# kfirc1503/generative-audio

Hardware: AMD Instinct MI355X
Metric: spectrogram-frames/sec, NPPC K=5 FullSubNet+ train step (higher is better)
Workload: dtype bf16

## Files before the change

generative-audio_amd/csrc/tcn.hip:

```cpp
#include <cstdlib>
#include "common.h"
#include "mfma_tile.h"
#include "nppc_hip.h"

namespace {


template <typename T, int EPI>
__global__ __launch_bounds__(256) void gemm_nt_kernel(GemmArgs g) {
  const int ks = g.ksplit > 1 ? g.ksplit : 1;
  const int z = blockIdx.z / ks, ksl = blockIdx.z % ks;
  const T* A = reinterpret_cast<const T*>(g.A) + (size_t)z * g.strideA + (size_t)ksl * g.K;
  const T* B = reinterpret_cast<const T*>(g.B) + (size_t)z * g.strideB + (size_t)ksl * g.K;
  const int lane = threadIdx.x & 63, wave = threadIdx.x >> 6, n = lane & 15, q = lane >> 4;
  const int r0 = blockIdx.x * 128 + wave * 32, c0 = blockIdx.y * 64;
  const T* ap = A + (size_t)(r0 + n) * g.lda + 8 * q;
  const T* bp = B + (size_t)(c0 + n) * g.ldb + 8 * q;
  f32x4 acc[2][4];
  nt_reg_mainloop<T>(acc, g.K / 32, g.lda, g.ldb, [&](int kk) { return ap + 32 * kk; }, [&](int kk) { return bp + 32 * kk; },
                     g.relu_in);

  const NtEpilogue<T, EPI> ep(g, z, blockIdx.x * 128);
  float s1 = 0.f, s2 = 0.f;
#pragma unroll
// ... 488 lines not shown

extern "C" int nppc_gemm_nt_splitk(int prec, const void* A, long lda, const void* B, long ldb, float* C, long ldc, int M, int N,
                                   long K, int ksplit, void* stream) {
  if (!A || !B || !C || M <= 0 || N <= 0 || K <= 0 || ksplit < 1) return NPPC_EBADARG;
  const int bk = prec == NPPC_PREC_BF16 ? 64 : 32;
  if (M % 128 || N % 128 || K % ((long)bk * ksplit) || lda % 8 || ldb % 8) return NPPC_EUNSUPPORTED;
  dim3 grid(M / 128, N / 128, ksplit);
  LAUNCH_T(prec, gemm_nt_tiled_kernel, grid, (const TT*)A, lda, (const TT*)B, ldb, C, ldc, (long)M * ldc, K / ksplit);
  return NPPC_OK;
}

namespace {

typedef __attribute__((ext_vector_type(4))) short s16x4;

template <int BN>
__global__ __launch_bounds__(256, 2) void gemm_tn_tiled_kernel(const bf16_t* __restrict__ A, long lda, const bf16_t* __restrict__ B,
                                                               long ldb, float* __restrict__ C, long ldc, long slab_stride,
                                                               long Rz, int ntap, int Wp, int shift_a, int nzb, long bsA,
                                                               long bsB, long bsC) {
  constexpr int BM = 128, BR = 64, NT = 2 * BM;
  constexpr int RSA = BM + 8, RSB = BN + 8;
  constexpr int WN = BN / 2;
  constexpr int NJ = WN / 16;
  __shared__ __attribute__((aligned(16))) bf16_t lds[2][BR * RSA + BR * RSB];
  const int tid = threadIdx.x, lane = tid & 63, wave = tid >> 6, i16 = lane & 15, qq = lane >> 4;
  const int wm = wave >> 1, wn = wave & 1;
  unsigned bx = blockIdx.x, by = blockIdx.y, bz = blockIdx.z;
  if (gridDim.z % 8 == 0) {
    const unsigned tiles = gridDim.x * gridDim.y;
    const unsigned lin = bx + gridDim.x * (by + gridDim.y * bz);
    const unsigned xcd = lin & 7, j = lin >> 3;
    bz = xcd + 8 * (j / tiles);
    const unsigned t = j % tiles;
    bx = t % gridDim.x;
    by = t / gridDim.x;
  }
  const unsigned bb = bz / nzb;
  bz %= nzb;
  A += (size_t)bb * bsA;
  B += (size_t)bb * bsB;
  C += (size_t)bb * bsC;
  const long m0 = (long)bx * BM, n0 = (long)by * BN;
  const int ksl = nzb / ntap, tap = bz / ksl;
  const long rbase = (long)(bz % ksl) * Rz;
  const long boff = ntap == 9 ? (long)(tap / 3 - 1) * Wp + (tap % 3 - 1) : 0;
  const bf16_t* Ab = A + (rbase + (shift_a ? boff : 0)) * lda + m0;
  const bf16_t* Bb = B + (rbase + (shift_a ? 0 : boff)) * ldb + n0;
  float* Cz = C + (size_t)bz * slab_stride;

  constexpr int ACH = BM / 8, BCH = BN / 8;
  constexpr int NA = BR * ACH / NT, NB = BR * BCH / NT;
  static_assert(NA == 4 && (NB == 4 || NB == 2 || NB == 1), "staging slots are named registers");
  const int arow = tid / ACH, ac = tid % ACH, brow = tid / BCH, bc = tid % BCH;
  constexpr int ASTEP = NT / ACH, BSTEP = NT / BCH;
  const bf16_t* gA = Ab + (long)arow * lda + ac * 8;
  const bf16_t* gB = Bb + (long)brow * ldb + bc * 8;
  const int sA = arow * RSA + ac * 8, sB = BR * RSA + brow * RSB + bc * 8;
  uint4 ra0, ra1, ra2, ra3, rb0, rb1 = {}, rb2 = {}, rb3 = {};
#define TN_GLOAD(r0)                                                            \
  ra0 = *reinterpret_cast<const uint4*>(gA + ((r0) + 0 * ASTEP) * lda);         \
  ra1 = *reinterpret_cast<const uint4*>(gA + ((r0) + 1 * ASTEP) * lda);         \
  ra2 = *reinterpret_cast<const uint4*>(gA + ((r0) + 2 * ASTEP) * lda);         \
  ra3 = *reinterpret_cast<const uint4*>(gA + ((r0) + 3 * ASTEP) * lda);         \
  rb0 = *reinterpret_cast<const uint4*>(gB + ((r0) + 0 * BSTEP) * ldb);         \
  if (NB >= 2) rb1 = *reinterpret_cast<const uint4*>(gB + ((r0) + 1 * BSTEP) * ldb); \
  if (NB == 4) {                                                                \
    rb2 = *reinterpret_cast<const uint4*>(gB + ((r0) + 2 * BSTEP) * ldb);       \
    rb3 = *reinterpret_cast<const uint4*>(gB + ((r0) + 3 * BSTEP) * ldb);       \
  }
#define TN_LSTORE(buf)                                                          \
  *reinterpret_cast<uint4*>(&lds[buf][sA + 0 * ASTEP * RSA]) = ra0;             \
  *reinterpret_cast<uint4*>(&lds[buf][sA + 1 * ASTEP * RSA]) = ra1;             \
  *reinterpret_cast<uint4*>(&lds[buf][sA + 2 * ASTEP * RSA]) = ra2;             \
  *reinterpret_cast<uint4*>(&lds[buf][sA + 3 * ASTEP * RSA]) = ra3;             \
  *reinterpret_cast<uint4*>(&lds[buf][sB + 0 * BSTEP * RSB]) = rb0;             \
  if (NB >= 2) *reinterpret_cast<uint4*>(&lds[buf][sB + 1 * BSTEP * RSB]) = rb1; \
  if (NB == 4) {                                                                \
    *reinterpret_cast<uint4*>(&lds[buf][sB + 2 * BSTEP * RSB]) = rb2;           \
    *reinterpret_cast<uint4*>(&lds[buf][sB + 3 * BSTEP * RSB]) = rb3;           \
  }
  auto tfrag = [&](const bf16_t* tile, int rs, int r0, int col0) -> bf16x8 {
    const int q4 = i16 >> 2, p4 = i16 & 3;
    const bf16_t* base = tile + (r0 + 8 * qq + q4) * rs + col0 + 4 * p4;
    const s16x4 lo = __builtin_amdgcn_ds_read_tr16_b64_v4i16((__attribute__((address_space(3))) s16x4*)(base));
    const s16x4 hi = __builtin_amdgcn_ds_read_tr16_b64_v4i16((__attribute__((address_space(3))) s16x4*)(base + 4 * rs));
    typedef __attribute__((ext_vector_type(8))) short s16x8;
    s16x8 v = {lo[0], lo[1], lo[2], lo[3], hi[0], hi[1], hi[2], hi[3]};
    return __builtin_bit_cast(bf16x8, v);
  };

  f32x4 acc[4][NJ];
#pragma unroll
  for (int i = 0; i < 4; ++i)
#pragma unroll
    for (int j = 0; j < NJ; ++j) acc[i][j] = f32x4{0.f, 0.f, 0.f, 0.f};

  const long nstage = Rz / BR;
  TN_GLOAD(0)
  TN_LSTORE(0)
  __syncthreads();
  for (long s = 0; s < nstage; ++s) {
    const int buf = (int)(s & 1);
    if (s + 1 < nstage) { TN_GLOAD((s + 1) * BR) }
    const bf16_t* ta = lds[buf];
    const bf16_t* tb = lds[buf] + BR * RSA;
#pragma unroll
    for (int ks = 0; ks < BR / 32; ++ks) {
      bf16x8 af[4], bfr[NJ];
#pragma unroll
      for (int i = 0; i < 4; ++i) af[i] = tfrag(ta, RSA, 32 * ks, wm * 64 + 16 * i);
#pragma unroll
      for (int j = 0; j < NJ; ++j) bfr[j] = tfrag(tb, RSB, 32 * ks, wn * WN + 16 * j);
#pragma unroll
      for (int i = 0; i < 4; ++i)
#pragma unroll
        for (int j = 0; j < NJ; ++j) acc[i][j] = mma16(af[i], bfr[j], acc[i][j]);
    }
    if (s + 1 < nstage) { TN_LSTORE(buf ^ 1) }
    __syncthreads();
  }
#undef TN_GLOAD
#undef TN_LSTORE
#pragma unroll
  for (int i = 0; i < 4; ++i)
#pragma unroll
    for (int j = 0; j < NJ; ++j)
#pragma unroll
      for (int r = 0; r < 4; ++r) {
        const long row = m0 + wm * 64 + 16 * i + 4 * qq + r;
        const long col = n0 + wn * WN + 16 * j + i16;
        Cz[row * ldc + col] = acc[i][j][r];
      }
}

}

namespace {
constexpr int DR_BM = 256;

__device__ __forceinline__ int dr_key(int row, int nch) {
  const int k = (row & 3) | (((row >> 3) & 1) << 2);
  return nch >= 8 ? k : (k & (nch - 1));
}
__device__ __forceinline__ int dr_phys(int bytes_in_row, int key, int nch) {
  const int c = bytes_in_row >> 5;
  int pc = c + key;
  if (pc >= nch) pc -= nch;
// ... 132 lines not shown
    for (int j = 0; j < NJ; ++j)
#pragma unroll
      for (int r = 0; r < 4; ++r) {
        const long row = m0 + wm * (BM / 4) + 16 * i + 4 * qq + r;
        const long col = c0 + wn * (BN / 2) + 16 * j + i16;
        Cz[row * ldc + col] = acc[i][j][r];
      }
  if (do_rowsum && i16 == 0) {
#pragma unroll
    for (int i = 0; i < MI; ++i)
#pragma unroll
      for (int r = 0; r < 4; ++r) rs[m0 + wm * (BM / 4) + 16 * i + 4 * qq + r] = racc[i][r];
  }
}

__device__ __forceinline__ void dr_xcd_remap(unsigned& bx, unsigned& by, unsigned& bz) {
  if (gridDim.z % 8 == 0) {
    const unsigned tiles = gridDim.x * gridDim.y;
    const unsigned lin = bx + gridDim.x * (by + gridDim.y * bz);
    const unsigned xcd = lin & 7, j = lin >> 3;
    bz = xcd + 8 * (j / tiles);
    const unsigned t = j % tiles;
    bx = t % gridDim.x;
    by = t / gridDim.x;
  }
}

template <int BN, int BR, int STAGES>
__global__ __launch_bounds__(512, 1) void gemm_tn_dma_kernel(const bf16_t* __restrict__ A, long lda, const bf16_t* __restrict__ B,
                                                             long ldb, float* __restrict__ C, long ldc, long slab_stride, long Rz,
                                                             int nzb, long bsA, long bsB, long bsC, float* __restrict__ rowsum,
                                                             int ntap, int Wp, int shift_a) {
  unsigned bx = blockIdx.x, by = blockIdx.y, bz = blockIdx.z;
  dr_xcd_remap(bx, by, bz);
  const unsigned bb = bz / nzb;
  bz %= nzb;
  A += (size_t)bb * bsA;
  B += (size_t)bb * bsB;
  C += (size_t)bb * bsC;
  const int ksl = nzb / ntap, tap = bz / ksl;
  const long boff = ntap == 9 ? (long)(tap / 3 - 1) * Wp + (tap % 3 - 1) : 0;
  const long rbase = (long)(bz % ksl) * Rz;
  float* rs = rowsum != nullptr && by == 0 ? rowsum + ((size_t)bb * nzb + bz) * ((size_t)gridDim.x * DR_BM) : nullptr;
  dma_tile<DR_BM, BN, BR, STAGES>(A, lda, B, ldb, C + (size_t)bz * slab_stride, ldc, (long)bx * DR_BM, (long)by * BN, (long)by * BN,
                           rbase + (shift_a ? boff : 0), rbase + (shift_a ? 0 : boff), Rz, rs);
}

template <int BM, int BR, int STAGES>
__global__ __launch_bounds__(512, 1) void gemm_tn_dma2_kernel(const bf16_t* __restrict__ A, long lda, const bf16_t* __restrict__ B1,
                                                              long ldb1, int nt1, const bf16_t* __restrict__ B2, long ldb2, int N2,
                                                              float* __restrict__ C, long ldc, long slab_stride, long Rz,
                                                              float* __restrict__ rowsum) {
  unsigned bx = blockIdx.x, by = blockIdx.y, bz = blockIdx.z;
  dr_xcd_remap(bx, by, bz);
  const long m0 = (long)bx * BM, rbase = (long)bz * Rz;
  float* Cz = C + (size_t)bz * slab_stride;
  float* rs = rowsum != nullptr && by == 0 ? rowsum + (size_t)bz * ((size_t)gridDim.x * BM) : nullptr;
  if ((int)by >= nt1 && N2 == 64) {
    dma_tile<BM, 64, BR, STAGES>(A, lda, B2, ldb2, Cz, ldc, m0, 0, (long)nt1 * 192, rbase, rbase, Rz, nullptr);
    return;
  }
  const bool second = (int)by >= nt1;
  const long n0 = (long)(second ? by - nt1 : by) * 192;
  dma_tile<BM, 192, BR, STAGES>(A, lda, second ? B2 : B1, second ? ldb2 : ldb1, Cz, ldc, m0, n0, (long)by * 192, rbase, rbase, Rz, rs);
}

}

static int launch_tn(const void* A, long lda, const void* B, long ldb, float* C, long ldc, int M, int N, long R, int ksplit,
// ... 88 lines not shown
      return NPPC_ELAUNCH;
    attr = true;
  }
  hipLaunchKernelGGL((gemm_tn_dma2_kernel<DR_BM, 32, 5>), dim3(M / DR_BM, nt1 + nt2, ksplit), dim3(512), smem, s, (const bf16_t*)A,
                     lda, (const bf16_t*)B1, ldb1, nt1, (const bf16_t*)B2, ldb2, N2, C, ldc, (long)M * ldc, R / ksplit, rowsum);
  NPPC_CHECK_LAUNCH();
  return NPPC_OK;
}

extern "C" int nppc_gemm_tn_splitk_batched(const void* A, long lda, long sA, const void* B, long ldb, long sB, float* C, long ldc,
                                           long sC, int M, int N, long R, int ksplit, int batch, void* stream) {
  if (batch < 1) return NPPC_EBADARG;
  return launch_tn(A, lda, B, ldb, C, ldc, M, N, R, ksplit, 1, 0, 0, stream, batch, sA, sB, sC);
}

extern "C" int nppc_gemm_tn_splitk_taps(const void* A, long lda, const void* B, long ldb, float* C, long ldc, int M, int N,
                                        long R, int ksplit, int Wp, int shift_a, void* stream) {
  return launch_tn(A, lda, B, ldb, C, ldc, M, N, R, ksplit, 9, Wp, shift_a, stream);
}
```

generative-audio_amd/nppc_audio/_hip.py:

```python
import ctypes
import os
import threading

import torch

_HERE = os.path.dirname(os.path.abspath(__file__))
LIB_PATH = os.path.join(_HERE, "libnppc_hip.so")

PREC_BF16 = 0
PREC_F32 = 1
_ERR = {1: "bad argument", 2: "kernel launch failed", 3: "unsupported shape/configuration"}

_lib = None

c_p = ctypes.c_void_p
c_i = ctypes.c_int
c_l = ctypes.c_long
c_f = ctypes.c_float


def lib():
    global _lib
    if _lib is None:
        if not os.path.exists(LIB_PATH):
# ... 17 lines not shown


def stream():
    return c_p(torch.cuda.current_stream().cuda_stream)


def check(rc, what):
    if rc != 0:
        raise RuntimeError(f"{what} failed: {_ERR.get(rc, rc)}")


def ptr_array(tensors):
    for t in tensors:
        assert t.is_cuda and t.is_contiguous()
    return (ctypes.c_void_p * len(tensors))(*[t.data_ptr() for t in tensors])


def mid_bwd_part_elems(B, C, Tp, batch):
    n = c_l()
    call("nppc_tcn_mid_bwd_part_elems", B, C, Tp, batch, ctypes.byref(n))
    return n.value


def conv_thin_part_elems():
    n = c_l()
    call("nppc_conv_thin_part_elems", ctypes.byref(n))
    return n.value


def masked_mse_work_elems():
# ... 57 lines not shown
                           I, I, I, I, I, I, P],
    "nppc_scale_transpose": [I, P, P, P, I, I, I, I, I, I, P],
    "nppc_gemm_nt": [I, I, P, L, L, P, L, L, P, L, L, P, L, P, L, L, P, L, P, L, I, I, I, I, I, I, I, I, I, P],
    "nppc_tcn_mid_bwd_part_elems": [I, I, I, I, PL],
    "nppc_tcn_mid_bwd": [I, P, P, P, P, P, P, P, P, P, P, P, P, P, P, P, P, P, P, P, P, P, P, P, P, P, P, I, I, I, P,
                         I, I, I, I, I, F, L, L, L, I, I, P],
    "nppc_tcn_mid_bwd_finish": [P, L, P, L, I, I, I, P, P, P, P, P, P, P, P, P, P, I, I, L, L, I, I, P],
    "nppc_gemm_nt_colsum": [I, I, P, L, L, P, L, L, P, L, L, P, L, P, L, L, I, I, I, I, I, I, I, P, P],
    "nppc_gemm_nt_gn": [I, P, L, L, P, L, L, P, L, L, P, P, L, P, L, L, P, L, D, F, I, I, I, I, I, I, I, P],
    "nppc_tcn_pack_sconv": [I, P, P, P, P, P, P, P, I, I, I, I, I, I, L, L, L, L, P],
    "nppc_gemm_nt_splitk": [I, P, L, P, L, P, L, I, I, L, I, P],
    "nppc_gemm_tn_splitk": [P, L, P, L, P, L, I, I, L, I, P],
    "nppc_gemm_tn_splitk_rowsum": [P, L, P, L, P, L, I, I, L, I, P, P],
    "nppc_gemm_tn_splitk2": [P, L, P, L, I, P, L, I, P, L, I, L, I, P, P],
    "nppc_gemm_tn_splitk_batched": [P, L, L, P, L, L, P, L, L, I, I, L, I, I, P],
    "nppc_reduce_slabs_t": [P, I, L, L, P, L, I, I, L, L, I, P],
    "nppc_gemm_tn_splitk_taps": [P, L, P, L, P, L, I, I, L, I, I, I, P],
    "nppc_tcn_dwconv": [I, P, P, P, P, P, P, P, P, P, I, I, I, I, I, I, F, L, L, L, I, P],
    "nppc_tcn_gn_apply": [I, P, P, P, P, P, I, I, I, I, I, F, L, L, L, I, P],
    "nppc_pack_matrix": [I, P, P, I, I, I, I, I, P],
    "nppc_pack_matrix_batched": [I, P, P, I, I, I, I, I, I, I, L, L, L, L, P],
    "nppc_subband_mean": [I, P, I, P, I, L, P, P, P, I, I, I, I, I, P],
    "nppc_subband_stage": [I, P, I, P, I, L, P, P, I, I, I, I, I, I, I, I, P],
    "nppc_sb_head": [I, P, P, P, P, L, I, I, I, I, I, P],
    "nppc_gram": [P, P, P, P, P, I, I, L, P],
    "nppc_combine": [P, P, P, P, P, P, P, I, I, L, P],
    "nppc_gs_solve": [P, P, P, I, I, I, P],
    "nppc_gs_bwd_solve": [P, P, P, P, I, I, I, P],
    "nppc_loss_solve": [P, P, P, P, P, P, P, P, P, P, I, I, P],
    "nppc_loss_bwd_coef": [P, P, P, F, F, P, I, I, P],
# ... 176 lines not shown
```

generative-audio_amd/nppc_audio/engine.py:

```python
import ctypes

import numpy as np
import torch

from . import _hip as H
from .ops_lstm import (PackedLSTM, PackedLSTMBwd, ROW_PAD, WGRAD_SPLITS, bwd_head_fusable, forward_x_ld, lstm2_backward, lstm2_forward,
                       own_workspaces, padded_rows,
                       rows_view, workspace)

TCN_HIDDEN = 512
TCN_DILATIONS = (1, 2, 5, 9, 1, 2, 5, 9)
BRANCHES = ("", "_real", "_imag")
EPI_PLAIN, EPI_PRELU_STATS, EPI_RESIDUAL, EPI_RELU, EPI_PLAIN_F32, EPI_MASK_POS = 0, 1, 2, 3, 4, 5


def rup(a, b):
    return (a + b - 1) // b * b


TCN_WGRAD_SPLITS = 8
TCN_WGRAD_MAIN_BLOCKS = 1


class FlatParams:

    def __init__(self, module, device):
        named = list(module.named_parameters())
        total = sum(p.numel() for _, p in named)
        self.flat = torch.empty(total, dtype=torch.float32, device=device)
        self.grad = None
        self.off = {}
        o = 0
        for n, p in named:
            k = p.numel()
            self.flat[o:o + k].copy_(p.detach().reshape(-1))
            p.data = self.flat[o:o + k].view(p.shape)
# ... 63 lines not shown
        self.F, self.nm, self.O = num_freqs, n_maps, out_size
        self.nb, self.la, self.Hd, self.G = sb_neighbors, look_ahead, sb_hidden, groups
        self.ks = tuple(kersize)
        self.prec = prec
        self.dt = H.dtype_of(prec)
        self.trainable = trainable
        self.C = n_maps * num_freqs
        self.ldC = rup(self.C, 64)
        self.ldF = rup(num_freqs, 64)
        self.KC = self.ldC
        self.dev = flat.flat.device
        self.I = 2 * sb_neighbors + 1 + 3
        self.sP = flat.branch_stride()
        self.sAtt = flat.attention_stride()
        self.packed_version = None
        self._side = None
        self._gen = 0
        self.last_train = None
        self.grad_range_hook = None
        self.early_buckets_ok = self._check_bucket_layout() if trainable else False
        self.pre_lstm_hook = None
        self.defer_join = False
        self.join_pending = False
        self.bufs = {}
        own_workspaces(self)
        self.lstm = PackedLSTM(self.I, self.Hd, prec, self.dev)
        self.KX = self.lstm.kx
        self.mult = torch.from_numpy(unfold_multiplicity(self.F, self.nb)).to(self.dev)
        C, ldC, ldF = self.C, self.ldC, self.ldF
        self.W1p = torch.zeros(8, 3, TCN_HIDDEN, ldC, dtype=self.dt, device=self.dev)
# ... 227 lines not shown
            self.last_train = d
        return out

    def _grad_buffer(self):
        first = self.fp.named[0][1]
        for k in (0, 1):
            if self.gbuf[k] is None:
                self.gbuf[k] = torch.empty_like(self.fp.flat)
            if first.grad is None or first.grad.data_ptr() != self.gbuf[k].data_ptr():
                self.fp.grad = self.gbuf[k]
                return self.gbuf[k]
        raise RuntimeError("unreachable")

    def g(self, name):
        return self.fp.gview(name)

    def _wgrad(self, AT, lda, sA, BT, ldb, sB, rows, ncolsN, K, S, dst_name_or_tensor, dst_ld, out_rows, ncols, slab,
               batch=1, sDst=0, permH=0, col0=0, accumulate=0):
        s = H.stream()
        dst = self.g(dst_name_or_tensor) if isinstance(dst_name_or_tensor, str) else dst_name_or_tensor
        bk = 64 if self.prec == H.PREC_BF16 else 32
        if batch == 1 and rows % 128 == 0 and ncolsN % 128 == 0 and K % (bk * S) == 0:
            H.call("nppc_gemm_nt_splitk", self.prec, AT, lda, BT, ldb, slab, ncolsN, rows, ncolsN, K, S, s)
        else:
            H.call("nppc_gemm_nt", self.prec, EPI_PLAIN_F32, AT, lda, sA, BT, ldb, sB, slab, ncolsN, rows * ncolsN, None,
                   0, None, 0, 0, None, 0, None, 0, rows, ncolsN, K, rows, rows, ncolsN, 0, batch, S, s)
        H.call("nppc_reduce_slabs", slab, S, rows * ncolsN, ncolsN, dst, dst_ld, out_rows, col0, ncols, permH, accumulate,
               S * rows * ncolsN, sDst, batch, s)

    def _lstm_wgrad(self, dg1, dg2, x_rows, h1_rows, h2_rows, Tv, Nseq, head=None, guards=None):
# ... 130 lines not shown
        self._side.wait_stream(main)
        with torch.cuda.stream(self._side):
            self._lstm_wgrad(dg1, dg2, d["x_rows"], lo["h1_rows"], lo["h2_rows"], Tv, Nseq, head=head_wgrad,
                             guards=(lo["h1_guard"], lo["h2_guard"]) if "h1_guard" in lo else None)
            if self.grad_range_hook is not None and self.early_buckets_ok:
                self.grad_range_hook(G, self.fp.off["sb_model.sequence_model.weight_ih_l0"][0], G.numel())
        dpre_fb = ws("dpre_fb", (3, B, Tp, ldF), zero=True)
        Dsb = ws("Dsb", (B,), torch.float64)
        H.call("nppc_subband_stage_bwd", prec, dx, d["x_tm"], d["fb"], d["sbscale"], Dsb, dpre_fb, B, F, Tp, Tv, ldF, R * ldF,
               self.nb, self.G, self.KX, s)
        S2 = TCN_WGRAD_SPLITS if R % (64 * TCN_WGRAD_SPLITS) == 0 else (8 if R % (32 * 8) == 0 else 1)
        Fr = rup(F, 128)
        Cr = rup(ldC, 128)
        tA = ws("tA", (3, max(Cr, TCN_HIDDEN, Fr), R), zero=True)
        tB = ws("tB", (3, max(ldC, TCN_HIDDEN), R), zero=True)
        slab2 = ws("slab2", (3 * S2 * max(Cr * TCN_HIDDEN, TCN_HIDDEN * ldC, Fr * ldC),), torch.float32)
        X8 = d["X"][8]
        sTA, sTB = tA.shape[1] * R, tB.shape[1] * R

        def on_side(fn):
            ev = torch.cuda.Event()
            ev.record(main)
            with torch.cuda.stream(self._side):
                self._side.wait_event(ev)
                fn()

        def fc_wgrad(slab):
            q = H.stream()
            H.colsum(prec, dpre_fb, self.g("fb_model.fc_output_layer.bias"), R, F, ldF, R * ldF, sP, 3,
                     lambda n: ws("cs_fc", (n,), torch.float32), q)
            H.call("nppc_transpose", prec, dpre_fb, tA, R, F, ldF, R, R * ldF, sTA, 0, 3, q)
            H.call("nppc_transpose", prec, X8, tB, R, ldC, ldC, R, R * ldC, sTB, 1, 3, q)
            self._wgrad(tA, R, sTA, tB, R, sTB, Fr, ldC, R, S2, "fb_model.fc_output_layer.weight", C, F, C, slab, batch=3, sDst=sP)
        tn_ok = prec == H.PREC_BF16 and TCN_HIDDEN % 128 == 0 and ldC % 64 == 0 and R % (64 * S2) == 0
        if not tn_ok:
            fc_wgrad(slab2)
        if tn_ok:
            dXL = [ws(f"dX_{i}", (3, B, Tp, ldC)) for i in range(9)]
            a2L = [ws(f"a2_{i}", (3, B, Tp, TCN_HIDDEN), zero=True) for i in range(8)]
            h2L = [ws(f"h2b_{i}", (3, B, Tp, TCN_HIDDEN)) for i in range(8)]
            dXa, dXb = dXL[8], dXL[7]
        else:
            dXa = ws("dXa", (3, B, Tp, ldC))
            dXb = ws("dXb", (3, B, Tp, ldC))

        bk = 64 if prec == H.PREC_BF16 else 32
        cs_ok = tn_ok and ldF % bk == 0 and TCN_HIDDEN % bk == 0
        cp_all = ws("colpart", (8, 3, R // 128, ldC), torch.float32) if cs_ok else None
        cpL = [cp_all[i] for i in range(8)] if cs_ok else None
        if cs_ok:
            H.call("nppc_gemm_nt_colsum", prec, EPI_MASK_POS, dpre_fb, ldF, R * ldF, self.WfcT, ldF, ldC * ldF, dXa, ldC, R * ldC,
                   None, 0, X8, ldC, R * ldC, R, ldC, ldF, Tp, Tv, C, 3, cpL[7], s)
        else:
            H.call("nppc_gemm_nt", prec, EPI_MASK_POS, dpre_fb, ldF, R * ldF, self.WfcT, ldF, ldC * ldF, dXa, ldC, R * ldC, None, 0,
                   X8, ldC, R * ldC, None, 0, None, 0, R, ldC, ldF, Tp, Tv, C, 0, 3, 1, s)
        sAct = B * Tp * TCN_HIDDEN
# ... 26 lines not shown
                H.colsum(prec, dXo, self.g(pre + "sconv.bias"), R, C, ldC, R * ldC, sP, 3,
                         lambda n: ws("cs_sconv", (n,), torch.float32), s)
            H.call("nppc_gemm_nt", prec, EPI_PLAIN, dXo, ldC, R * ldC, self.W2T[i], ldC, TCN_HIDDEN * ldC, h1b, TCN_HIDDEN,
                   sAct, None, 0, None, 0, 0, None, 0, None, 0, R, TCN_HIDDEN, ldC, Tp, Tv, TCN_HIDDEN, 0, 3, 1, s)
            H.call("nppc_tcn_mid_bwd", prec, h1b, y2, y1, st1, st2, Smid, Pmid[i], self.p(pre + "norm1.weight"), self.p(pre + "norm1.bias"),
                   self.p(pre + "norm2.weight"), self.p(pre + "norm2.bias"), self.p(pre + "depthwise_conv.weight"),
                   self.p(pre + "prelu1.weight"), self.p(pre + "prelu2.weight"), a2, h2b, self.g(pre + "norm2.weight"),
                   self.g(pre + "norm2.bias"), self.g(pre + "norm1.weight"), self.g(pre + "norm1.bias"),
                   self.g(pre + "depthwise_conv.weight"), self.g(pre + "depthwise_conv.bias"), self.g(pre + "prelu1.weight"),
                   self.g(pre + "prelu2.weight"), self.g(pre + "conv1x1.bias"),
                   cpL[i] if cs_ok else None, R // 128, ldC, C, self.g(pre + "sconv.bias") if cs_ok else None,
                   B, TCN_HIDDEN, Tp, Tv, dil, 1e-8, sAct, B * 2, sP, 3, 0, s)
            if i == 4 and early:
                finish_mid(4, 8)
            if tn_ok:
                inline = i < TCN_WGRAD_MAIN_BLOCKS
                wslab = ws("slab_main", (3 * S2 * TCN_HIDDEN * ldC,), torch.float32) if inline else slab2

                def sconv_wgrad(a2=a2, dXo=dXo, dest=self.g(pre + "sconv.weight"), wslab=wslab):
                    q = H.stream()
                    H.call("nppc_gemm_tn_splitk_batched", a2, TCN_HIDDEN, sAct, dXo, ldC, R * ldC, wslab, ldC,
                           S2 * TCN_HIDDEN * ldC, TCN_HIDDEN, ldC, R, S2, 3, q)
                    H.call("nppc_reduce_slabs_t", wslab, S2, TCN_HIDDEN * ldC, ldC, dest, TCN_HIDDEN, C, TCN_HIDDEN,
                           S2 * TCN_HIDDEN * ldC, sP, 3, q)
                if inline:
                    sconv_wgrad()
                else:
                    on_side(sconv_wgrad)
            else:
                H.call("nppc_transpose", prec, dXo, tA, R, ldC, ldC, R, R * ldC, sTA, 0, 3, s)
                H.call("nppc_transpose", prec, a2, tB, R, TCN_HIDDEN, TCN_HIDDEN, R, sAct, sTB, 0, 3, s)
                self._wgrad(tA, R, sTA, tB, R, sTB, Cr, TCN_HIDDEN, R, S2, pre + "sconv.weight", TCN_HIDDEN, C, TCN_HIDDEN,
                            slab2, batch=3, sDst=sP)
            if tn_ok:
                def c1_wgrad(h2b=h2b, Xin=Xin, dest=self.g(pre + "conv1x1.weight"), wslab=wslab):
                    q = H.stream()
                    H.call("nppc_gemm_tn_splitk_batched", h2b, TCN_HIDDEN, sAct, Xin, ldC, R * ldC, wslab, ldC,
                           S2 * TCN_HIDDEN * ldC, TCN_HIDDEN, ldC, R, S2, 3, q)
                    H.call("nppc_reduce_slabs", wslab, S2, TCN_HIDDEN * ldC, ldC, dest, C, TCN_HIDDEN, 0, C, 0, 0,
                           S2 * TCN_HIDDEN * ldC, sP, 3, q)
                if inline:
                    c1_wgrad()
                else:
                    on_side(c1_wgrad)
            else:
                H.call("nppc_transpose", prec, h2b, tA, R, TCN_HIDDEN, TCN_HIDDEN, R, sAct, sTA, 0, 3, s)
                H.call("nppc_transpose", prec, Xin, tB, R, ldC, ldC, R, R * ldC, sTB, 0, 3, s)
                self._wgrad(tA, R, sTA, tB, R, sTB, TCN_HIDDEN, ldC, R, S2, pre + "conv1x1.weight", C, TCN_HIDDEN, C, slab2,
                            batch=3, sDst=sP)
            if cs_ok and i > 0:
                H.call("nppc_gemm_nt_colsum", prec, EPI_RESIDUAL, h2b, TCN_HIDDEN, sAct, self.W1T[i], TCN_HIDDEN, ldC * TCN_HIDDEN,
                       dXi, ldC, R * ldC, None, 0, dXo, ldC, R * ldC, R, ldC, TCN_HIDDEN, Tp, Tv, C, 3, cpL[i - 1], s)
            else:
                H.call("nppc_gemm_nt", prec, EPI_RESIDUAL, h2b, TCN_HIDDEN, sAct, self.W1T[i], TCN_HIDDEN, ldC * TCN_HIDDEN, dXi, ldC,
                       R * ldC, None, 0, dXo, ldC, R * ldC, None, 0, None, 0, R, ldC, TCN_HIDDEN, Tp, Tv, C, 0, 3, 1, s)
            dXo, dXi = dXi, dXo
            if i == 4 and self.grad_range_hook is not None and self.early_buckets_ok:
                def blocks_done():
                    for br in BRANCHES:
                        a = self.fp.off[f"fb_model{br}.sequence_model.4.conv1x1.weight"][0]
# ... 56 lines not shown
```

include/nppc_hip.h:

```cpp
#ifndef NPPC_HIP_H
#define NPPC_HIP_H
#ifdef __cplusplus
extern "C" {
#endif

int nppc_stft(const float* wave, float* re, float* im, float* mag , int B, int L, int nfft, int hop,
              void* stream);
int nppc_dropband(const float* in, float* out, int B, int C, int F, int T, int G, void* stream);
int nppc_cirm_build_compress(const float* nr, const float* ni, const float* cr, const float* ci, float* out, int B, int F,
                             int T, int G, float eps, void* stream);
int nppc_cirm_decompress_apply_conj(const float* crm, const float* nr, const float* ni, float* dec ,
                                    float* emag, float* ere, float* eim, int B, int F, int T, void* stream);

int nppc_cirm_decompress_apply(const float* crm, const float* nr, const float* ni, float* dec , float* emag,
                               float* ere, float* eim, int B, int F, int T, void* stream);
int nppc_istft(const float* re, const float* im, float* out, int B, int T, int nfft, int hop, int L, void* stream);

int nppc_rowsum(const float* x, double* sums, long R, int T, void* stream);
int nppc_tsse_fwd_maps(int prec, const float* const* maps, int nmaps, double* rowsum, const float* cw0, const float* cb0,
                       const float* cw1, const float* cb1, const float* cw2, const float* cb2, int ks0, int ks1, int ks2,
                       const float* fcw, const float* fcb, const float* w1, const float* b1, const float* w2, const float* b2, long sW,
                       float* scale, float* ns, float* pre, float* sq, float* h1, float* sg, void* X0, long sY, int B, int C, int T,
                       int look_ahead, int Tp, int ld, void* stream);
int nppc_tsse_bwd_ws_elems(int nmaps, int B, int C, int ks0, int ks1, int ks2, long* elems);
// ... 19 lines not shown

int nppc_gemm_nt(int prec, int epi, const void* A, long lda, long sA, const void* B, long ldb, long sB, void* C, long ldc,
                 long sC, const float* bias, long sBias, const void* res, long ldres, long sRes, const float* slope,
                 long sSlope, double* stats, long sStats, int R, int N, int K, int Tp, int Tv, int Nv, int relu_in,
                 int batch, int ksplit, void* stream);
int nppc_gemm_nt_splitk(int prec, const void* A, long lda, const void* B, long ldb, float* C, long ldc, int M, int N, long K,
                        int ksplit, void* stream);
int nppc_gemm_tn_splitk(const void* A, long lda, const void* B, long ldb, float* C, long ldc, int M, int N, long R, int ksplit,
                        void* stream);
int nppc_gemm_tn_splitk_rowsum(const void* A, long lda, const void* B, long ldb, float* C, long ldc, int M, int N, long R,
                               int ksplit, float* rowsum, void* stream);
int nppc_gemm_tn_splitk2(const void* A, long lda, const void* B1, long ldb1, int N1, const void* B2, long ldb2, int N2, float* C,
                         long ldc, int M, long R, int ksplit, float* rowsum, void* stream);
int nppc_gemm_tn_splitk_batched(const void* A, long lda, long sA, const void* B, long ldb, long sB, float* C, long ldc, long sC,
                                int M, int N, long R, int ksplit, int batch, void* stream);
int nppc_gemm_tn_splitk_taps(const void* A, long lda, const void* B, long ldb, float* C, long ldc, int M, int N, long R,
                             int ksplit, int Wp, int shift_a, void* stream);
int nppc_pack_matrix(int prec, const float* src, void* dst, int N, int K, int Npad, int ldd, int transpose, void* stream);
int nppc_pack_matrix_batched(int prec, const float* src, void* dst, int N, int K, int Npad, int ldd, int transpose, int n_a,
                             int n_b, long src_stride_a, long src_stride_b, long dst_stride_a, long dst_stride_b, void* stream);
int nppc_tcn_dwconv(int prec, const void* in, void* out, const double* st1, double* st2, const float* gamma,
                    const float* beta, const float* wd, const float* bd, const float* slope2, int B, int Cc, int ld, int Tp,
                    int Tv, int dil, float eps, long sAct, long sSt, long sP, int batch, void* stream);
int nppc_tcn_gn_apply(int prec, const void* in, void* out, const double* st, const float* gamma, const float* beta, int B,
                      int Cc, int ld, int Tp, int Tv, float eps, long sAct, long sSt, long sP, int batch, void* stream);
int nppc_tcn_gn_bwd(int prec, const void* dA, const void* y, const double* st, const float* gamma, const float* slope,
                    double* S, void* dpre, float* dgamma, float* dbeta, float* dslope, int B, int Cc, int Tp, int Tv, float eps,
                    long sAct, long sSt, long sP, int batch, void* stream);
int nppc_tcn_dwconv_bwd(int prec, const void* du, const void* y1, const double* st1, const float* gamma, const float* beta,
                        const float* wd, void* dz, float* dwd, float* dbd, int B, int Cc, int Tp, int Tv, int dil, float eps,
// ... 419 lines not shown
```

Before: 254,400.

## Batch TCN weight-gradient GEMMs into grouped kernel with direct fused stores

Adds a grouped TN GEMM kernel that takes a table of problems (A, B, destination, store kind) and computes many per-block sconv and conv1x1 weight gradients in one launch. It reduces over the full R in each block instead of using split-K slabs plus separate reduce kernels, and writes results straight to the parameter gradients, transposing through LDS when needed. Accumulation is blocked into chunked partial sums to limit fp32 error growth. The per-layer launches move to two grouped launches on the side stream, issued at block 4 and block 0. This cuts launch count and slab traffic, but with no split-K each block runs a long sequential reduction, so parallelism and overlap with the main backward change.

```diff
diff --git a/generative-audio_amd/csrc/tcn.hip b/generative-audio_amd/csrc/tcn.hip
--- a/generative-audio_amd/csrc/tcn.hip
+++ b/generative-audio_amd/csrc/tcn.hip
@@ -526,19 +526,10 @@
 
 typedef __attribute__((ext_vector_type(4))) short s16x4;
 
-template <int BN>
-__global__ __launch_bounds__(256, 2) void gemm_tn_tiled_kernel(const bf16_t* __restrict__ A, long lda, const bf16_t* __restrict__ B,
-                                                               long ldb, float* __restrict__ C, long ldc, long slab_stride,
-                                                               long Rz, int ntap, int Wp, int shift_a, int nzb, long bsA,
-                                                               long bsB, long bsC) {
-  constexpr int BM = 128, BR = 64, NT = 2 * BM;
-  constexpr int RSA = BM + 8, RSB = BN + 8;
-  constexpr int WN = BN / 2;
-  constexpr int NJ = WN / 16;
-  __shared__ __attribute__((aligned(16))) bf16_t lds[2][BR * RSA + BR * RSB];
-  const int tid = threadIdx.x, lane = tid & 63, wave = tid >> 6, i16 = lane & 15, qq = lane >> 4;
-  const int wm = wave >> 1, wn = wave & 1;
-  unsigned bx = blockIdx.x, by = blockIdx.y, bz = blockIdx.z;
+constexpr int TT_BM = 128, TT_BR = 64;
+template <int BN> constexpr int tt_stage_elems() { return TT_BR * (TT_BM + 8) + TT_BR * (BN + 8); }
+
+__device__ __forceinline__ void tn_xcd_remap(unsigned& bx, unsigned& by, unsigned& bz) {
   if (gridDim.z % 8 == 0) {
     const unsigned tiles = gridDim.x * gridDim.y;
     const unsigned lin = bx + gridDim.x * (by + gridDim.y * bz);
@@ -548,6 +539,128 @@
     bx = t % gridDim.x;
     by = t / gridDim.x;
   }
+}
+
+template <int BN, bool BLOCKED = false>
+__device__ __forceinline__ void tn_tiled_mainloop(f32x4 (&acc)[4][BN / 32], bf16_t* lds, const bf16_t* __restrict__ Ab, long lda,
+                                                  const bf16_t* __restrict__ Bb, long ldb, long nstage, long chunk = 0) {
+  constexpr int BM = TT_BM, BR = TT_BR, NT = 2 * BM;
+  constexpr int RSA = BM + 8, RSB = BN + 8;
+  constexpr int WN = BN / 2;
+  constexpr int NJ = WN / 16;
+  constexpr int STAGE = tt_stage_elems<BN>();
+  const int tid = threadIdx.x, lane = tid & 63, wave = tid >> 6, i16 = lane & 15, qq = lane >> 4;
+  const int wm = wave >> 1, wn = wave & 1;
+
+  constexpr int ACH = BM / 8, BCH = BN / 8;
+  constexpr int NA = BR * ACH / NT, NB = BR * BCH / NT;
+  static_assert(NA == 4 && (NB == 4 || NB == 2 || NB == 1), "staging slots are named registers");
+  const int arow = tid / ACH, ac = tid % ACH, brow = tid / BCH, bc = tid % BCH;
+  constexpr int ASTEP = NT / ACH, BSTEP = NT / BCH;
+  const bf16_t* gA = Ab + (long)arow * lda + ac * 8;
+  const bf16_t* gB = Bb + (long)brow * ldb + bc * 8;
+  const int sA = arow * RSA + ac * 8, sB = BR * RSA + brow * RSB + bc * 8;
+  typedef const __attribute__((address_space(1))) u32x4* tn_gvec;
+  u32x4 ra0, ra1, ra2, ra3, rb0, rb1 = {}, rb2 = {}, rb3 = {};
+#define TN_GLOAD(r0)                                                            \
+  ra0 = *(tn_gvec)(gA + ((r0) + 0 * ASTEP) * lda);         \
+  ra1 = *(tn_gvec)(gA + ((r0) + 1 * ASTEP) * lda);         \
+  ra2 = *(tn_gvec)(gA + ((r0) + 2 * ASTEP) * lda);         \
+  ra3 = *(tn_gvec)(gA + ((r0) + 3 * ASTEP) * lda);         \
+  rb0 = *(tn_gvec)(gB + ((r0) + 0 * BSTEP) * ldb);         \
+  if (NB >= 2) rb1 = *(tn_gvec)(gB + ((r0) + 1 * BSTEP) * ldb); \
+  if (NB == 4) {                                                                \
+    rb2 = *(tn_gvec)(gB + ((r0) + 2 * BSTEP) * ldb);       \
+    rb3 = *(tn_gvec)(gB + ((r0) + 3 * BSTEP) * ldb);       \
+  }
+#define TN_LSTORE(buf)                                                          \
+  *reinterpret_cast<u32x4*>(&lds[(buf) * STAGE + sA + 0 * ASTEP * RSA]) = ra0;             \
+  *reinterpret_cast<u32x4*>(&lds[(buf) * STAGE + sA + 1 * ASTEP * RSA]) = ra1;             \
+  *reinterpret_cast<u32x4*>(&lds[(buf) * STAGE + sA + 2 * ASTEP * RSA]) = ra2;             \
+  *reinterpret_cast<u32x4*>(&lds[(buf) * STAGE + sA + 3 * ASTEP * RSA]) = ra3;             \
+  *reinterpret_cast<u32x4*>(&lds[(buf) * STAGE + sB + 0 * BSTEP * RSB]) = rb0;             \
+  if (NB >= 2) *reinterpret_cast<u32x4*>(&lds[(buf) * STAGE + sB + 1 * BSTEP * RSB]) = rb1; \
+  if (NB == 4) {                                                                \
+    *reinterpret_cast<u32x4*>(&lds[(buf) * STAGE + sB + 2 * BSTEP * RSB]) = rb2;           \
+    *reinterpret_cast<u32x4*>(&lds[(buf) * STAGE + sB + 3 * BSTEP * RSB]) = rb3;           \
+  }
+  auto tfrag = [&](const bf16_t* tile, int rs, int r0, int col0) -> bf16x8 {
+    const int q4 = i16 >> 2, p4 = i16 & 3;
+    const bf16_t* base = tile + (r0 + 8 * qq + q4) * rs + col0 + 4 * p4;
+    const s16x4 lo = __builtin_amdgcn_ds_read_tr16_b64_v4i16((__attribute__((address_space(3))) s16x4*)(base));
+    const s16x4 hi = __builtin_amdgcn_ds_read_tr16_b64_v4i16((__attribute__((address_space(3))) s16x4*)(base + 4 * rs));
+    typedef __attribute__((ext_vector_type(8))) short s16x8;
+    s16x8 v = {lo[0], lo[1], lo[2], lo[3], hi[0], hi[1], hi[2], hi[3]};
+    return __builtin_bit_cast(bf16x8, v);
+  };
+
+#pragma unroll
+  for (int i = 0; i < 4; ++i)
+#pragma unroll
+    for (int j = 0; j < NJ; ++j) acc[i][j] = f32x4{0.f, 0.f, 0.f, 0.f};
+  f32x4 tot[BLOCKED ? 4 : 1][NJ];
+#pragma unroll
+  for (int i = 0; i < (BLOCKED ? 4 : 1); ++i)
+#pragma unroll
+    for (int j = 0; j < NJ; ++j) tot[i][j] = f32x4{0.f, 0.f, 0.f, 0.f};
+  long left = chunk;
+
+  TN_GLOAD(0)
+  TN_LSTORE(0)
+  __syncthreads();
+  for (long s = 0; s < nstage; ++s) {
+    const int buf = (int)(s & 1);
+    if (s + 1 < nstage) { TN_GLOAD((s + 1) * BR) }
+    const bf16_t* ta = lds + buf * STAGE;
+    const bf16_t* tb = ta + BR * RSA;
+#pragma unroll
+    for (int ks = 0; ks < BR / 32; ++ks) {
+      bf16x8 af[4], bfr[NJ];
+#pragma unroll
+      for (int i = 0; i < 4; ++i) af[i] = tfrag(ta, RSA, 32 * ks, wm * 64 + 16 * i);
+#pragma unroll
+      for (int j = 0; j < NJ; ++j) bfr[j] = tfrag(tb, RSB, 32 * ks, wn * WN + 16 * j);
+#pragma unroll
+      for (int i = 0; i < 4; ++i)
+#pragma unroll
+        for (int j = 0; j < NJ; ++j) acc[i][j] = mma16(af[i], bfr[j], acc[i][j]);
+    }
+    if constexpr (BLOCKED) {
+      if (--left == 0) {
+        left = chunk;
+#pragma unroll
+        for (int i = 0; i < 4; ++i)
+#pragma unroll
+          for (int j = 0; j < NJ; ++j) {
+            tot[i][j] += acc[i][j];
+            acc[i][j] = f32x4{0.f, 0.f, 0.f, 0.f};
+          }
+      }
+    }
+    if (s + 1 < nstage) { TN_LSTORE(buf ^ 1) }
+    __syncthreads();
+  }
+#undef TN_GLOAD
+#undef TN_LSTORE
+  if constexpr (BLOCKED) {
+#pragma unroll
+    for (int i = 0; i < 4; ++i)
+#pragma unroll
+      for (int j = 0; j < NJ; ++j) acc[i][j] = tot[i][j];
+  }
+}
+
+template <int BN>
+__global__ __launch_bounds__(256, 2) void gemm_tn_tiled_kernel(const bf16_t* __restrict__ A, long lda, const bf16_t* __restrict__ B,
+                                                               long ldb, float* __restrict__ C, long ldc, long slab_stride,
+                                                               long Rz, int ntap, int Wp, int shift_a, int nzb, long bsA,
+                                                               long bsB, long bsC) {
+  constexpr int BM = TT_BM, WN = BN / 2, NJ = WN / 16;
+  __shared__ __attribute__((aligned(16))) bf16_t lds[2 * tt_stage_elems<BN>()];
+  const int lane = threadIdx.x & 63, wave = threadIdx.x >> 6, i16 = lane & 15, qq = lane >> 4;
+  const int wm = wave >> 1, wn = wave & 1;
+  unsigned bx = blockIdx.x, by = blockIdx.y, bz = blockIdx.z;
+  tn_xcd_remap(bx, by, bz);
   const unsigned bb = bz / nzb;
   bz %= nzb;
   A += (size_t)bb * bsA;
@@ -560,80 +673,8 @@
   const bf16_t* Ab = A + (rbase + (shift_a ? boff : 0)) * lda + m0;
   const bf16_t* Bb = B + (rbase + (shift_a ? 0 : boff)) * ldb + n0;
   float* Cz = C + (size_t)bz * slab_stride;
-
-  constexpr int ACH = BM / 8, BCH = BN / 8;
-  constexpr int NA = BR * ACH / NT, NB = BR * BCH / NT;
-  static_assert(NA == 4 && (NB == 4 || NB == 2 || NB == 1), "staging slots are named registers");
-  const int arow = tid / ACH, ac = tid % ACH, brow = tid / BCH, bc = tid % BCH;
-  constexpr int ASTEP = NT / ACH, BSTEP = NT / BCH;
-  const bf16_t* gA = Ab + (long)arow * lda + ac * 8;
-  const bf16_t* gB = Bb + (long)brow * ldb + bc * 8;
-  const int sA = arow * RSA + ac * 8, sB = BR * RSA + brow * RSB + bc * 8;
-  uint4 ra0, ra1, ra2, ra3, rb0, rb1 = {}, rb2 = {}, rb3 = {};
-#define TN_GLOAD(r0)                                                            \
-  ra0 = *reinterpret_cast<const uint4*>(gA + ((r0) + 0 * ASTEP) * lda);         \
-  ra1 = *reinterpret_cast<const uint4*>(gA + ((r0) + 1 * ASTEP) * lda);         \
-  ra2 = *reinterpret_cast<const uint4*>(gA + ((r0) + 2 * ASTEP) * lda);         \
-  ra3 = *reinterpret_cast<const uint4*>(gA + ((r0) + 3 * ASTEP) * lda);         \
-  rb0 = *reinterpret_cast<const uint4*>(gB + ((r0) + 0 * BSTEP) * ldb);         \
-  if (NB >= 2) rb1 = *reinterpret_cast<const uint4*>(gB + ((r0) + 1 * BSTEP) * ldb); \
-  if (NB == 4) {                                                                \
-    rb2 = *reinterpret_cast<const uint4*>(gB + ((r0) + 2 * BSTEP) * ldb);       \
-    rb3 = *reinterpret_cast<const uint4*>(gB + ((r0) + 3 * BSTEP) * ldb);       \
-  }
-#define TN_LSTORE(buf)                                                          \
-  *reinterpret_cast<uint4*>(&lds[buf][sA + 0 * ASTEP * RSA]) = ra0;             \
-  *reinterpret_cast<uint4*>(&lds[buf][sA + 1 * ASTEP * RSA]) = ra1;             \
-  *reinterpret_cast<uint4*>(&lds[buf][sA + 2 * ASTEP * RSA]) = ra2;             \
-  *reinterpret_cast<uint4*>(&lds[buf][sA + 3 * ASTEP * RSA]) = ra3;             \
-  *reinterpret_cast<uint4*>(&lds[buf][sB + 0 * BSTEP * RSB]) = rb0;             \
-  if (NB >= 2) *reinterpret_cast<uint4*>(&lds[buf][sB + 1 * BSTEP * RSB]) = rb1; \
-  if (NB == 4) {                                                                \
-    *reinterpret_cast<uint4*>(&lds[buf][sB + 2 * BSTEP * RSB]) = rb2;           \
-    *reinterpret_cast<uint4*>(&lds[buf][sB + 3 * BSTEP * RSB]) = rb3;           \
-  }
-  auto tfrag = [&](const bf16_t* tile, int rs, int r0, int col0) -> bf16x8 {
-    const int q4 = i16 >> 2, p4 = i16 & 3;
-    const bf16_t* base = tile + (r0 + 8 * qq + q4) * rs + col0 + 4 * p4;
-    const s16x4 lo = __builtin_amdgcn_ds_read_tr16_b64_v4i16((__attribute__((address_space(3))) s16x4*)(base));
-    const s16x4 hi = __builtin_amdgcn_ds_read_tr16_b64_v4i16((__attribute__((address_space(3))) s16x4*)(base + 4 * rs));
-    typedef __attribute__((ext_vector_type(8))) short s16x8;
-    s16x8 v = {lo[0], lo[1], lo[2], lo[3], hi[0], hi[1], hi[2], hi[3]};
-    return __builtin_bit_cast(bf16x8, v);
-  };
-
   f32x4 acc[4][NJ];
-#pragma unroll
-  for (int i = 0; i < 4; ++i)
-#pragma unroll
-    for (int j = 0; j < NJ; ++j) acc[i][j] = f32x4{0.f, 0.f, 0.f, 0.f};
-
-  const long nstage = Rz / BR;
-  TN_GLOAD(0)
-  TN_LSTORE(0)
-  __syncthreads();
-  for (long s = 0; s < nstage; ++s) {
-    const int buf = (int)(s & 1);
-    if (s + 1 < nstage) { TN_GLOAD((s + 1) * BR) }
-    const bf16_t* ta = lds[buf];
-    const bf16_t* tb = lds[buf] + BR * RSA;
-#pragma unroll
-    for (int ks = 0; ks < BR / 32; ++ks) {
-      bf16x8 af[4], bfr[NJ];
-#pragma unroll
-      for (int i = 0; i < 4; ++i) af[i] = tfrag(ta, RSA, 32 * ks, wm * 64 + 16 * i);
-#pragma unroll
-      for (int j = 0; j < NJ; ++j) bfr[j] = tfrag(tb, RSB, 32 * ks, wn * WN + 16 * j);
-#pragma unroll
-      for (int i = 0; i < 4; ++i)
-#pragma unroll
-        for (int j = 0; j < NJ; ++j) acc[i][j] = mma16(af[i], bfr[j], acc[i][j]);
-    }
-    if (s + 1 < nstage) { TN_LSTORE(buf ^ 1) }
-    __syncthreads();
-  }
-#undef TN_GLOAD
-#undef TN_LSTORE
+  tn_tiled_mainloop<BN>(acc, lds, Ab, lda, Bb, ldb, Rz / TT_BR);
 #pragma unroll
   for (int i = 0; i < 4; ++i)
 #pragma unroll
@@ -644,6 +685,48 @@
         const long col = n0 + wn * WN + 16 * j + i16;
         Cz[row * ldc + col] = acc[i][j][r];
       }
+}
+
+template <int BN>
+__device__ __forceinline__ void tn_grouped_tile(const nppc_tn_problem& p, bf16_t* lds, int m0, int n0, long nstage, long chunk) {
+  constexpr int BM = TT_BM, WN = BN / 2, NJ = WN / 16;
+  constexpr int EP = BN + 1;
+  static_assert(BM * EP * 4 <= 2 * tt_stage_elems<BN>() * 2, "the fp32 tile fits into the operand buffers");
+  const int tid = threadIdx.x, lane = tid & 63, wave = tid >> 6, i16 = lane & 15, qq = lane >> 4;
+  const int wm = wave >> 1, wn = wave & 1;
+  f32x4 acc[4][NJ];
+  tn_tiled_mainloop<BN, true>(acc, lds, (const bf16_t*)p.A + m0, p.lda, (const bf16_t*)p.B + n0, p.ldb, nstage, chunk);
+  float* tile = reinterpret_cast<float*>(lds);
+#pragma unroll
+  for (int i = 0; i < 4; ++i)
+#pragma unroll
+    for (int j = 0; j < NJ; ++j)
+#pragma unroll
+      for (int r = 0; r < 4; ++r) tile[(wm * 64 + 16 * i + 4 * qq + r) * EP + wn * WN + 16 * j + i16] = acc[i][j][r];
+  __syncthreads();
+  const int nv = (int)p.nvalid - n0;
+  __attribute__((address_space(1))) float* dst = (__attribute__((address_space(1))) float*)p.dst;
+  if (p.kind == NPPC_TN_STORE_TRANSPOSED) {
+    for (int e = tid; e < BM * BN; e += 256) {
+      const int n = e / BM, m = e % BM;
+      if (n < nv) dst[(long)(n0 + n) * p.dst_ld + m0 + m] = tile[m * EP + n];
+    }
+  } else {
+    for (int e = tid; e < BM * BN; e += 256) {
+      const int m = e / BN, n = e % BN;
+      if (n < nv) dst[(long)(m0 + m) * p.dst_ld + n0 + n] = tile[m * EP + n];
+    }
+  }
+}
+
+__global__ __launch_bounds__(256, 2) void gemm_tn_grouped_kernel(const nppc_tn_problem* __restrict__ table, long R,
+                                                                 long chunk, int nwide) {
+  __shared__ __attribute__((aligned(16))) bf16_t lds[2 * tt_stage_elems<128>()];
+  unsigned bx = blockIdx.x, by = blockIdx.y, bz = blockIdx.z;
+  tn_xcd_remap(bx, by, bz);
+  const nppc_tn_problem p = table[bz];
+  if ((int)by < nwide) tn_grouped_tile<128>(p, lds, (int)bx * TT_BM, (int)by * 128, R / TT_BR, chunk);
+  else tn_grouped_tile<64>(p, lds, (int)bx * TT_BM, nwide * 128, R / TT_BR, chunk);
 }
 
 }
@@ -806,25 +889,13 @@
   }
 }
 
-__device__ __forceinline__ void dr_xcd_remap(unsigned& bx, unsigned& by, unsigned& bz) {
-  if (gridDim.z % 8 == 0) {
-    const unsigned tiles = gridDim.x * gridDim.y;
-    const unsigned lin = bx + gridDim.x * (by + gridDim.y * bz);
-    const unsigned xcd = lin & 7, j = lin >> 3;
-    bz = xcd + 8 * (j / tiles);
-    const unsigned t = j % tiles;
-    bx = t % gridDim.x;
-    by = t / gridDim.x;
-  }
-}
-
 template <int BN, int BR, int STAGES>
 __global__ __launch_bounds__(512, 1) void gemm_tn_dma_kernel(const bf16_t* __restrict__ A, long lda, const bf16_t* __restrict__ B,
                                                              long ldb, float* __restrict__ C, long ldc, long slab_stride, long Rz,
                                                              int nzb, long bsA, long bsB, long bsC, float* __restrict__ rowsum,
                                                              int ntap, int Wp, int shift_a) {
   unsigned bx = blockIdx.x, by = blockIdx.y, bz = blockIdx.z;
-  dr_xcd_remap(bx, by, bz);
+  tn_xcd_remap(bx, by, bz);
   const unsigned bb = bz / nzb;
   bz %= nzb;
   A += (size_t)bb * bsA;
@@ -844,7 +915,7 @@
                                                               float* __restrict__ C, long ldc, long slab_stride, long Rz,
                                                               float* __restrict__ rowsum) {
   unsigned bx = blockIdx.x, by = blockIdx.y, bz = blockIdx.z;
-  dr_xcd_remap(bx, by, bz);
+  tn_xcd_remap(bx, by, bz);
   const long m0 = (long)bx * BM, rbase = (long)bz * Rz;
   float* Cz = C + (size_t)bz * slab_stride;
   float* rs = rowsum != nullptr && by == 0 ? rowsum + (size_t)bz * ((size_t)gridDim.x * BM) : nullptr;
@@ -963,6 +1034,18 @@
   return launch_tn(A, lda, B, ldb, C, ldc, M, N, R, ksplit, 1, 0, 0, stream, batch, sA, sB, sC);
 }
 
+extern "C" int nppc_gemm_tn_grouped(const nppc_tn_problem* table, int nprob, int M, int N, long R, void* stream) {
+  if (!table || nprob < 1 || M <= 0 || N <= 0 || R <= 0) return NPPC_EBADARG;
+  if (M % TT_BM || N % 64 || R % TT_BR || nprob > 65535) return NPPC_EUNSUPPORTED;
+  const long nstage = R / TT_BR;
+  int nblk = 8;
+  while (nstage % nblk) --nblk;
+  hipLaunchKernelGGL(gemm_tn_grouped_kernel, dim3(M / TT_BM, N / 128 + (N % 128 != 0), nprob), dim3(256), 0, (hipStream_t)stream,
+                     table, R, nstage / nblk, N / 128);
+  NPPC_CHECK_LAUNCH();
+  return NPPC_OK;
+}
+
 extern "C" int nppc_gemm_tn_splitk_taps(const void* A, long lda, const void* B, long ldb, float* C, long ldc, int M, int N,
                                         long R, int ksplit, int Wp, int shift_a, void* stream) {
   return launch_tn(A, lda, B, ldb, C, ldc, M, N, R, ksplit, 9, Wp, shift_a, stream);
diff --git a/generative-audio_amd/nppc_audio/_hip.py b/generative-audio_amd/nppc_audio/_hip.py
--- a/generative-audio_amd/nppc_audio/_hip.py
+++ b/generative-audio_amd/nppc_audio/_hip.py
@@ -55,6 +55,22 @@
     for t in tensors:
         assert t.is_cuda and t.is_contiguous()
     return (ctypes.c_void_p * len(tensors))(*[t.data_ptr() for t in tensors])
+
+
+TN_STORE_ASIS, TN_STORE_TRANSPOSED = 0, 1
+
+
+def tn_problem_table(problems, M, N, R):
+    rows = []
+    for A, lda, B, ldb, dst, dst_ld, nvalid, kind in problems:
+        assert A.is_cuda and B.is_cuda and dst.is_cuda and A.dtype == B.dtype == torch.bfloat16 and dst.dtype == torch.float32
+        assert lda % 8 == 0 and ldb % 8 == 0 and lda >= M and ldb >= N and A.data_ptr() % 16 == 0 and B.data_ptr() % 16 == 0
+        assert (R - 1) * lda + M <= A.numel() and (R - 1) * ldb + N <= B.numel() and 0 <= nvalid <= N
+        assert kind in (TN_STORE_ASIS, TN_STORE_TRANSPOSED)
+        n_rows, n_cols = (M, nvalid) if kind == TN_STORE_ASIS else (nvalid, M)
+        assert dst_ld >= n_cols and (n_rows - 1) * dst_ld + n_cols <= dst.numel()
+        rows.append([A.data_ptr(), lda, B.data_ptr(), ldb, dst.data_ptr(), dst_ld, nvalid, kind])
+    return torch.tensor(rows, dtype=torch.int64).to(problems[0][0].device)
 
 
 def mid_bwd_part_elems(B, C, Tp, batch):
@@ -142,6 +158,7 @@
     "nppc_gemm_tn_splitk_rowsum": [P, L, P, L, P, L, I, I, L, I, P, P],
     "nppc_gemm_tn_splitk2": [P, L, P, L, I, P, L, I, P, L, I, L, I, P, P],
     "nppc_gemm_tn_splitk_batched": [P, L, L, P, L, L, P, L, L, I, I, L, I, I, P],
+    "nppc_gemm_tn_grouped": [P, I, I, I, L, P],
     "nppc_reduce_slabs_t": [P, I, L, L, P, L, I, I, L, L, I, P],
     "nppc_gemm_tn_splitk_taps": [P, L, P, L, P, L, I, I, L, I, I, I, P],
     "nppc_tcn_dwconv": [I, P, P, P, P, P, P, P, P, P, I, I, I, I, I, I, F, L, L, L, I, P],
diff --git a/generative-audio_amd/nppc_audio/engine.py b/generative-audio_amd/nppc_audio/engine.py
--- a/generative-audio_amd/nppc_audio/engine.py
+++ b/generative-audio_amd/nppc_audio/engine.py
@@ -19,7 +19,6 @@
 
 
 TCN_WGRAD_SPLITS = 8
-TCN_WGRAD_MAIN_BLOCKS = 1
 
 
 class FlatParams:
@@ -113,6 +112,7 @@
         self.sP = flat.branch_stride()
         self.sAtt = flat.attention_stride()
         self.packed_version = None
+        self._tn_tables = {}
         self._side = None
         self._gen = 0
         self.last_train = None
@@ -370,6 +370,22 @@
 
     def g(self, name):
         return self.fp.gview(name)
+
+    def _tcn_wgrad_tables(self, G, d, dXL, a2L, h2L, R, blocks):
+        key = (G.data_ptr(), d["X"].data_ptr(), a2L[0].data_ptr(), R, blocks)
+        tabs = self._tn_tables.get(key)
+        if tabs is None:
+            C, ldC = self.C, self.ldC
+            sc, c1 = [], []
+            for i in blocks:
+                for z, br in enumerate(BRANCHES):
+                    pre = f"fb_model{br}.sequence_model.{i}."
+                    sc.append((a2L[i][z], TCN_HIDDEN, dXL[i + 1][z], ldC, self.g(pre + "sconv.weight"), TCN_HIDDEN, C,
+                               H.TN_STORE_TRANSPOSED))
+                    c1.append((h2L[i][z], TCN_HIDDEN, d["X"][i][z], ldC, self.g(pre + "conv1x1.weight"), C, C, H.TN_STORE_ASIS))
+            tabs = (H.tn_problem_table(sc, TCN_HIDDEN, ldC, R), H.tn_problem_table(c1, TCN_HIDDEN, ldC, R))
+            self._tn_tables[key] = tabs
+        return tabs
 
     def _wgrad(self, AT, lda, sA, BT, ldb, sB, rows, ncolsN, K, S, dst_name_or_tensor, dst_ld, out_rows, ncols, slab,
                batch=1, sDst=0, permH=0, col0=0, accumulate=0):
@@ -530,7 +546,6 @@
         Cr = rup(ldC, 128)
         tA = ws("tA", (3, max(Cr, TCN_HIDDEN, Fr), R), zero=True)
         tB = ws("tB", (3, max(ldC, TCN_HIDDEN), R), zero=True)
-        slab2 = ws("slab2", (3 * S2 * max(Cr * TCN_HIDDEN, TCN_HIDDEN * ldC, Fr * ldC),), torch.float32)
         X8 = d["X"][8]
         sTA, sTB = tA.shape[1] * R, tB.shape[1] * R
 
@@ -550,12 +565,19 @@
             self._wgrad(tA, R, sTA, tB, R, sTB, Fr, ldC, R, S2, "fb_model.fc_output_layer.weight", C, F, C, slab, batch=3, sDst=sP)
         tn_ok = prec == H.PREC_BF16 and TCN_HIDDEN % 128 == 0 and ldC % 64 == 0 and R % (64 * S2) == 0
         if not tn_ok:
+            slab2 = ws("slab2", (3 * S2 * max(Cr * TCN_HIDDEN, TCN_HIDDEN * ldC, Fr * ldC),), torch.float32)
             fc_wgrad(slab2)
         if tn_ok:
             dXL = [ws(f"dX_{i}", (3, B, Tp, ldC)) for i in range(9)]
             a2L = [ws(f"a2_{i}", (3, B, Tp, TCN_HIDDEN), zero=True) for i in range(8)]
             h2L = [ws(f"h2b_{i}", (3, B, Tp, TCN_HIDDEN)) for i in range(8)]
             dXa, dXb = dXL[8], dXL[7]
+
+            def tcn_wgrad(blocks):
+                sc_tab, c1_tab = self._tcn_wgrad_tables(G, d, dXL, a2L, h2L, R, blocks)
+                q = H.stream()
+                H.call("nppc_gemm_tn_grouped", sc_tab, sc_tab.shape[0], TCN_HIDDEN, ldC, R, q)
+                H.call("nppc_gemm_tn_grouped", c1_tab, c1_tab.shape[0], TCN_HIDDEN, ldC, R, q)
         else:
             dXa = ws("dXa", (3, B, Tp, ldC))
             dXb = ws("dXb", (3, B, Tp, ldC))
@@ -612,36 +634,14 @@
             if i == 4 and early:
                 finish_mid(4, 8)
             if tn_ok:
-                inline = i < TCN_WGRAD_MAIN_BLOCKS
-                wslab = ws("slab_main", (3 * S2 * TCN_HIDDEN * ldC,), torch.float32) if inline else slab2
-
-                def sconv_wgrad(a2=a2, dXo=dXo, dest=self.g(pre + "sconv.weight"), wslab=wslab):
-                    q = H.stream()
-                    H.call("nppc_gemm_tn_splitk_batched", a2, TCN_HIDDEN, sAct, dXo, ldC, R * ldC, wslab, ldC,
-                           S2 * TCN_HIDDEN * ldC, TCN_HIDDEN, ldC, R, S2, 3, q)
-                    H.call("nppc_reduce_slabs_t", wslab, S2, TCN_HIDDEN * ldC, ldC, dest, TCN_HIDDEN, C, TCN_HIDDEN,
-                           S2 * TCN_HIDDEN * ldC, sP, 3, q)
-                if inline:
-                    sconv_wgrad()
-                else:
-                    on_side(sconv_wgrad)
+                if i == 0 or (i == 4 and early):
+                    on_side(lambda blocks=tuple(range(3 if early and i == 0 else 7, i - 1, -1)): tcn_wgrad(blocks))
             else:
                 H.call("nppc_transpose", prec, dXo, tA, R, ldC, ldC, R, R * ldC, sTA, 0, 3, s)
                 H.call("nppc_transpose", prec, a2, tB, R, TCN_HIDDEN, TCN_HIDDEN, R, sAct, sTB, 0, 3, s)
                 self._wgrad(tA, R, sTA, tB, R, sTB, Cr, TCN_HIDDEN, R, S2, pre + "sconv.weight", TCN_HIDDEN, C, TCN_HIDDEN,
                             slab2, batch=3, sDst=sP)
-            if tn_ok:
-                def c1_wgrad(h2b=h2b, Xin=Xin, dest=self.g(pre + "conv1x1.weight"), wslab=wslab):
-                    q = H.stream()
-                    H.call("nppc_gemm_tn_splitk_batched", h2b, TCN_HIDDEN, sAct, Xin, ldC, R * ldC, wslab, ldC,
-                           S2 * TCN_HIDDEN * ldC, TCN_HIDDEN, ldC, R, S2, 3, q)
-                    H.call("nppc_reduce_slabs", wslab, S2, TCN_HIDDEN * ldC, ldC, dest, C, TCN_HIDDEN, 0, C, 0, 0,
-                           S2 * TCN_HIDDEN * ldC, sP, 3, q)
-                if inline:
-                    c1_wgrad()
-                else:
-                    on_side(c1_wgrad)
-            else:
+            if not tn_ok:
                 H.call("nppc_transpose", prec, h2b, tA, R, TCN_HIDDEN, TCN_HIDDEN, R, sAct, sTA, 0, 3, s)
                 H.call("nppc_transpose", prec, Xin, tB, R, ldC, ldC, R, R * ldC, sTB, 0, 3, s)
                 self._wgrad(tA, R, sTA, tB, R, sTB, TCN_HIDDEN, ldC, R, S2, pre + "conv1x1.weight", C, TCN_HIDDEN, C, slab2,
diff --git a/include/nppc_hip.h b/include/nppc_hip.h
--- a/include/nppc_hip.h
+++ b/include/nppc_hip.h
@@ -57,6 +57,15 @@
                          long ldc, int M, long R, int ksplit, float* rowsum, void* stream);
 int nppc_gemm_tn_splitk_batched(const void* A, long lda, long sA, const void* B, long ldb, long sB, float* C, long ldc, long sC,
                                 int M, int N, long R, int ksplit, int batch, void* stream);
+enum { NPPC_TN_STORE_ASIS = 0, NPPC_TN_STORE_TRANSPOSED = 1 };
+typedef struct nppc_tn_problem {
+  const void* A; long lda;
+  const void* B; long ldb;
+  float* dst; long dst_ld;
+  long nvalid;
+  long kind;
+} nppc_tn_problem;
+int nppc_gemm_tn_grouped(const nppc_tn_problem* table, int nprob, int M, int N, long R, void* stream);
 int nppc_gemm_tn_splitk_taps(const void* A, long lda, const void* B, long ldb, float* C, long ldc, int M, int N, long R,
                              int ksplit, int Wp, int shift_a, void* stream);
 int nppc_pack_matrix(int prec, const float* src, void* dst, int N, int K, int Npad, int ldd, int transpose, void* stream);
```

Result: faster. 257,000, median of 6 (+1.0%).
